# wuqianliang/Diff-Reg

Measured on AMD Instinct MI355X. Metric: scene-pairs/sec @ 20 denoise steps (N=M=256); IR/FMR parity vs ref, higher is better.
Workload: dtype f32; 1 GPU; cfg2: 3DMatch N=M=256, C=432, 20 denoise steps, max_condition_num=200 (warp active), 256 independent B=1 pairs per pass per GPU as 2 concurrent batch(es), one HIP-graph replay each on its own stream; pairs_per_pass_per_gpu=256, streams=2, denoise_steps=20, N=256, M=256, graph=True, parallelism=pairs sharded over 1 GPU(s)

## Files before the change

### diff-reg_amd/csrc/pgemm.hip

```cpp
#include <cstdlib>
#include <string.h>
#include <type_traits>
#include "pgemm.h"

namespace dr {
namespace {

typedef float f32x16 __attribute__((ext_vector_type(16)));
typedef float f32x2 __attribute__((ext_vector_type(2)));
typedef _Float16 f16x8 __attribute__((ext_vector_type(8)));
typedef _Float16 f16x2 __attribute__((ext_vector_type(2)));
typedef unsigned u32x4 __attribute__((ext_vector_type(4)));
typedef __attribute__((address_space(3))) void lds_void;
typedef const __attribute__((address_space(1))) void glb_void;

__device__ __forceinline__ void split2(float x0, float x1, unsigned& hi, unsigned& lo) {
    const f32x2 f = {x0, x1};
    const f16x2 h = __builtin_convertvector(f, f16x2);
    hi = __builtin_bit_cast(unsigned, h);
    const f32x2 hf = __builtin_convertvector(h, f32x2);
    const f32x2 r = {x0 - hf.x, x1 - hf.y};
    lo = __builtin_bit_cast(unsigned, __builtin_convertvector(r, f16x2));
}
__device__ __forceinline__ int scale_exp(float m) {
// ... 133 lines not shown
    const unsigned offBh = A_ST + (wn * BNW + l31) * 64 + ((h ^ sw) << 4), offBl = A_ST + (wn * BNW + l31) * 64 + (((2 + h) ^ sw) << 4);

    f32x16 acc[TNW];
#pragma unroll
    for (int j = 0; j < TNW; ++j)
#pragma unroll
        for (int r = 0; r < 16; ++r) acc[j][r] = 0.f;
    u32x4 fa0[2], fa1[2], fx[TNW / 2][2], fy[TNW - TNW / 2][2];
    f32x4 c16[M16 ? 4 : 1][M16 ? 7 : 1];

    auto run = [&](auto grp_t) __attribute__((always_inline)) {
        constexpr int GRP = decltype(grp_t)::value;
        constexpr bool EARLY = GRP == 0 && NST >= 4;
        constexpr int AHEAD = EARLY ? NST - 2 : NST - 1;
        constexpr bool ALL0 = NST >= 4 && WMN == 4;
        constexpr int AG = ALL0 ? 0 : 1;
        constexpr int WB_CNT = ALL0 ? 0 : (GG::NB + GG::NA) / 2 - GG::NA;
        constexpr int NW0 = GG::NB - WB_CNT;
        constexpr int NAP = GRP == AG ? 2 : 0;
        constexpr int NPIECE = GRP ? NAP + (WB_CNT + WMN - 1) / WMN : NAP + (NW0 + WMN - 1) / WMN;
        constexpr int NFULLP = GRP ? NAP + WB_CNT / WMN : NAP + NW0 / WMN;
        constexpr int PSTEP = (2 * NPIECE <= 3 * (TNW - TNW / 2)) ? 2 : 1;
        static_assert(EARLY || PSTEP * NPIECE <= 3 * (TNW - TNW / 2), "the DMA pieces of a stage must fit the gaps of the second burst");
        static_assert(!EARLY || NPIECE <= 3 * (TNW / 2), "... and those of the early group the gaps of the first");
        constexpr int REMP = GRP ? WB_CNT % WMN : NW0 % WMN;
        const int wl = w % WMN;
        const int st0 = GRP ? wl * (WB_CNT / WMN) + min(wl, WB_CNT % WMN) : WB_CNT + wl * (NW0 / WMN) + min(wl, NW0 % WMN);
        const unsigned voffW = lane * 16 + st0 * 1024, voffA = lane * 16 + 2 * wl * 1024;
        const char* ga = P.A0 + ((size_t)rb128 * P.nc0 + kbeg) * GG::A_IMG + sub * 64;
        const char* gb = P.W.img + ((size_t)nb * (P.nc0 + nc1) + kbeg) * GG::B_ST;
        const char* const ga1 = nc1 > 0 ? P.A1 + (size_t)rb128 * nc1 * GG::A_IMG + sub * 64 : nullptr;
        int ti = 0;
#define PG_DMA(ldsaddr, voff, gbase, imm)                                                                  \
    asm volatile("s_mov_b32 m0, %0\n\ts_nop 0\n\tglobal_load_lds_dwordx4 %1, %2 offset:%3" ::"s"(ldsaddr), "v"(voff), "s"(gbase), "i"(imm) : "memory")
        auto dma_piece = [&](int p, unsigned dstb) __attribute__((always_inline)) {
            const unsigned m0w = dstb + A_ST + st0 * 1024;
            const int pw = p - NAP;
            const unsigned hop = (unsigned)(pw >> 2) * 4096;
            if (p < NAP) PG_DMA(dstb + 2 * wl * 1024, voffA, ga, p * 1024);
            else if (pw < (GRP ? WB_CNT : NW0) / WMN || wl < (GRP ? WB_CNT : NW0) % WMN) PG_DMA(m0w + hop, voffW + hop, gb, (pw & 3) * 1024);
        };
        auto dma_advance = [&]() __attribute__((always_inline)) {
            ++ti;
            gb += GG::B_ST;
            ga = (ti == nc0) ? ga1 : ga + GG::A_IMG;
        };

        auto stage = [&](int s, auto steady_t, u32x4 (&ac)[2], u32x4 (&an)[2]) __attribute__((always_inline)) {
            constexpr bool STEADY = decltype(steady_t)::value;
            constexpr int NT1 = TNW / 2, NT2 = TNW - NT1, M1 = 3 * NT1;
            const unsigned sb = lds_base + (unsigned)(s % NST) * STAGE, sbn = lds_base + (unsigned)((s + 1) % NST) * STAGE;
            const unsigned Bh = sb + offBh, Bl = sb + offBl, Bhn = sbn + offBh, Bln = sbn + offBl;
            const bool has_next = STEADY || s + 1 < nst;
            const bool do_issue = STEADY || ti < nst;
            const unsigned dstb = lds_base + (unsigned)(ti % NST) * STAGE;
            if (s == nc0 && nc1 > 0) {
                const unsigned fb0 = lds_base + GG::WORK + (wm * 32 + 4 * h) * 4;
                u32x4 f[4];
                PG_READ(f[0], fb0, 0); PG_READ(f[1], fb0, 32); PG_READ(f[2], fb0, 64); PG_READ(f[3], fb0, 96);
                asm volatile("s_waitcnt lgkmcnt(0)" ::: "memory");
                __builtin_amdgcn_sched_barrier(0);
#pragma unroll
                for (int j = 0; j < TNW; ++j)
#pragma unroll
                    for (int r = 0; r < 16; ++r) acc[j][r] *= __uint_as_float(f[r >> 2][r & 3]);
                __builtin_amdgcn_sched_barrier(0);
            }
            auto gap = [&](int m) __attribute__((always_inline)) {
                {
                    if (m < NT2) {
                        PG_READ(fy[m][0], Bh, (NT1 + m) * 2048);
                        PG_READ(fy[m][1], Bl, (NT1 + m) * 2048);
                    } else if (m == M1 && has_next) {
                        PG_READ(an[0], sbn + offAh, 0);
                        PG_READ(an[1], sbn + offAl, 0);
                    } else if (m > M1 && m <= M1 + NT1 && has_next) {
                        PG_READ(fx[m - M1 - 1][0], Bhn, (m - M1 - 1) * 2048);
                        PG_READ(fx[m - M1 - 1][1], Bln, (m - M1 - 1) * 2048);
                    }
                }
                constexpr int MF = EARLY ? 0 : (PSTEP == 2 ? M1 + 1 : M1), STEP = EARLY ? 1 : PSTEP;
                if (m >= MF && m < MF + STEP * NPIECE && (m - MF) % STEP == 0) {
                    if (do_issue) dma_piece((m - MF) / STEP, dstb);
                    if ((m - MF) / STEP == NPIECE - 1 && do_issue) dma_advance();
                }
                if (m == M1 - 1) {
                    if (has_next) {
                        if (NST >= 4 && (STEADY || s + 2 < nst)) {
                            if (wl < REMP) PG_VMCNT(NFULLP + 1); else PG_VMCNT(NFULLP);
                        } else {
                            PG_VMCNT(0);
                        }
                    }
                    __builtin_amdgcn_s_barrier();
                    asm volatile("s_waitcnt lgkmcnt(0)" ::: "memory");
                }
            };
            const f16x8 ah = __builtin_bit_cast(f16x8, ac[0]), al = __builtin_bit_cast(f16x8, ac[1]);
#define PG_MFMA(X, Y, g)                                                        \
    acc[j] = __builtin_amdgcn_mfma_f32_32x32x16_f16(X, Y, acc[j], 0, 0, 0);      \
    __builtin_amdgcn_sched_barrier(0);                                          \
    gap(3 * j + g);                                                             \
    __builtin_amdgcn_sched_barrier(0);
            asm volatile("s_waitcnt lgkmcnt(0)" ::: "memory");
            __builtin_amdgcn_sched_barrier(0);
#pragma unroll
            for (int j = 0; j < NT1; ++j) {
                const f16x8 bh = __builtin_bit_cast(f16x8, fx[j][0]), bl = __builtin_bit_cast(f16x8, fx[j][1]);
                PG_MFMA(al, bh, 0)
                PG_MFMA(ah, bl, 1)
                PG_MFMA(ah, bh, 2)
            }
#pragma unroll
            for (int j = NT1; j < TNW; ++j) {
                const f16x8 bh = __builtin_bit_cast(f16x8, fy[j - NT1][0]), bl = __builtin_bit_cast(f16x8, fy[j - NT1][1]);
                PG_MFMA(al, bh, 0)
                PG_MFMA(ah, bl, 1)
                PG_MFMA(ah, bh, 2)
            }
#undef PG_MFMA
        };

#pragma unroll
        for (int q2 = 0; q2 < AHEAD; ++q2) {
            const unsigned dstb = lds_base + (unsigned)q2 * STAGE;
#pragma unroll
            for (int i = 0; i < NPIECE; ++i) dma_piece(i, dstb);
            dma_advance();
            if (q2 == 0) {
                __builtin_amdgcn_sched_barrier(0);
                stage_inputs();
                __builtin_amdgcn_sched_barrier(0);
                PG_VMCNT(0);
            }
        }
        __builtin_amdgcn_s_barrier();
        PG_READ(fa0[0], lds_base + offAh, 0);
        PG_READ(fa0[1], lds_base + offAl, 0);
#pragma unroll
        for (int j = 0; j < TNW / 2; ++j) {
            PG_READ(fx[j][0], lds_base + offBh, j * 2048);
            PG_READ(fx[j][1], lds_base + offBl, j * 2048);
        }
        int s = 0;
        for (; s + 1 < nst - (NST - 1); s += 2) {
            stage(s, std::true_type{}, fa0, fa1);
            stage(s + 1, std::true_type{}, fa1, fa0);
        }
        for (; s < nst; s += 2) {
            stage(s, std::false_type{}, fa0, fa1);
            if (s + 1 < nst) stage(s + 1, std::false_type{}, fa1, fa0);
        }
    };
    auto run16 = [&](auto iss_t) __attribute__((always_inline)) {
        constexpr bool ISS = decltype(iss_t)::value;
        const int l15 = lane & 15, g = lane >> 4, cs = g & 1, uh = g >> 1, sw16 = (l15 >> 2) & 3;
        const int wn4 = w & 3, wm2 = w >> 2;
        const unsigned oAh = cs * STAGE + (wm2 * 64 + l15) * 64 + ((uh ^ sw16) << 4), oAl = cs * STAGE + (wm2 * 64 + l15) * 64 + (((2 + uh) ^ sw16) << 4);
        const unsigned oBh = cs * STAGE + A_ST + (wn4 * 112 + l15) * 64 + ((uh ^ sw16) << 4), oBl = cs * STAGE + A_ST + (wn4 * 112 + l15) * 64 + (((2 + uh) ^ sw16) << 4);
#pragma unroll
        for (int i = 0; i < 4; ++i)
#pragma unroll
            for (int j = 0; j < 7; ++j) c16[i][j] = f32x4{0.f, 0.f, 0.f, 0.f};
        u32x4 fb[7][2], fa[2][2];
        const int nv0 = (nc0 + 1) & ~1, nvt = nv0 + ((nc1 + 1) & ~1), npair = nvt >> 1;
        const int z0 = (nc0 & 1) ? nv0 - 1 : -1, z1 = (nc1 & 1) ? nvt - 1 : -1;
        const int wl = w & 3, st0 = wl * 7;
        const unsigned voffW = lane * 16 + st0 * 1024, voffA = lane * 16 + 2 * wl * 1024;
        const char* ga = P.A0 + (size_t)rb128 * nc0 * GG::A_IMG + sub * 64;
        const char* gb = P.W.img + (size_t)nb * nst * GG::B_ST;
        const char* const ga1 = nc1 > 0 ? P.A1 + (size_t)rb128 * nc1 * GG::A_IMG + sub * 64 : nullptr;
        int ti = 0, tr = 0;
        auto piece = [&](int q) __attribute__((always_inline)) {
            if (ti == z0 || ti == z1) return;
            const unsigned dstb = lds_base + (unsigned)(ti % NST) * STAGE;
            const unsigned m0w = dstb + A_ST + st0 * 1024;
            const int pw = q - 2;
            const unsigned hop = (unsigned)(pw >> 2) * 4096;
            if (q < 2) PG_DMA(dstb + 2 * wl * 1024, voffA, ga, q * 1024);
            else PG_DMA(m0w + hop, voffW + hop, gb, (pw & 3) * 1024);
        };
        auto advance = [&]() __attribute__((always_inline)) {
            if (ti != z0 && ti != z1) {
                ++tr;
                gb += GG::B_ST;
                ga = (tr == nc0) ? ga1 : ga + GG::A_IMG;
            }
            ++ti;
        };
        auto stage = [&](int p, auto steady_t) __attribute__((always_inline)) {
            constexpr bool STEADY = decltype(steady_t)::value;
            const unsigned zm = ((2 * p + 1 == z0 || 2 * p + 1 == z1) && cs) ? 0u : ~0u;
            const unsigned sb = lds_base + (unsigned)(p & 1) * 2 * STAGE, sbn = lds_base + (unsigned)((p + 1) & 1) * 2 * STAGE;
            const bool has_next = STEADY || p + 1 < npair;
            if (2 * p == nv0 && nc1 > 0) {
#pragma unroll
                for (int i = 0; i < 4; ++i) {
                    const float f = s_fac[wm2 * 64 + 16 * i + l15];
#pragma unroll
                    for (int j = 0; j < 7; ++j) c16[i][j] *= f;
                }
                __builtin_amdgcn_sched_barrier(0);
            }
            auto gap = [&](int m) __attribute__((always_inline)) {
                const int pass = m / 21, gi = m % 21;
                if (pass < 3) {
                    if (gi == 0) PG_READ(fa[(pass + 1) & 1][0], sb + oAh, (pass + 1) * 1024);
                    if (gi == 1) PG_READ(fa[(pass + 1) & 1][1], sb + oAl, (pass + 1) * 1024);
                } else if (has_next) {
                    if (gi == 0) PG_READ(fa[0][0], sbn + oAh, 0);
                    if (gi == 1) PG_READ(fa[0][1], sbn + oAl, 0);
                    if (gi >= 1 && gi <= 7) PG_READ(fb[gi - 1][1], sbn + oBl, (gi - 1) * 1024);
                    if (gi >= 15 && gi <= 20) PG_READ(fb[gi - 15][0], sbn + oBh, (gi - 15) * 1024);
                    if (gi == 20) PG_READ(fb[6][0], sbn + oBh, 6 * 1024);
                }
                if (ISS) {
                    if (pass == 3 && gi >= 8 && gi <= 14) {
                        if (STEADY || ti < nvt) piece(gi - 8);
                    }
                    if (pass == 0 && gi % 3 == 2) {
                        const int q = 7 + gi / 3;
                        if (STEADY || ti < nvt) {
                            piece(q < 9 ? q : q - 9);
                            if (q == 8) advance();
                        }
                    }
                    if (pass == 1 && gi % 3 == 2 && gi <= 11) {
                        const int q = 14 + gi / 3;
                        if (STEADY || ti < nvt) {
                            piece(q - 9);
                            if (q == 17) advance();
                        }
                    }
                }
                if (pass == 2 && gi == 17) {
                    if (ISS && has_next) PG_VMCNT(0);
                    __builtin_amdgcn_s_barrier();
                }
            };
#define PG_MFMA16(X, Y, m)                                                              \
    c16[i][j] = __builtin_amdgcn_mfma_f32_16x16x32_f16(Y, X, c16[i][j], 0, 0, 0);       \
    __builtin_amdgcn_sched_barrier(0);                                                  \
    gap(m);                                                                             \
    __builtin_amdgcn_sched_barrier(0);
#pragma unroll
            for (int i = 0; i < 4; ++i) {
                if (i == 0) asm volatile("s_waitcnt lgkmcnt(7)" ::: "memory");
                else asm volatile("s_waitcnt lgkmcnt(0)" ::: "memory");
                __builtin_amdgcn_sched_barrier(0);
                const u32x4 a_h = fa[i & 1][0] & zm, a_l = fa[i & 1][1] & zm;
                const f16x8 ah = __builtin_bit_cast(f16x8, a_h), al = __builtin_bit_cast(f16x8, a_l);
#pragma unroll
                for (int j = 0; j < 7; ++j) { PG_MFMA16(ah, __builtin_bit_cast(f16x8, fb[j][1]), 21 * i + j) }
                if (i == 0) { asm volatile("s_waitcnt lgkmcnt(2)" ::: "memory"); __builtin_amdgcn_sched_barrier(0); }
#pragma unroll
                for (int j = 0; j < 7; ++j) { PG_MFMA16(al, __builtin_bit_cast(f16x8, fb[j][0]), 21 * i + 7 + j) }
#pragma unroll
                for (int j = 0; j < 7; ++j) { PG_MFMA16(ah, __builtin_bit_cast(f16x8, fb[j][0]), 21 * i + 14 + j) }
            }
#undef PG_MFMA16
        };
        if (ISS) {
#pragma unroll
            for (int q = 0; q < 9; ++q) piece(q);
            advance();
#pragma unroll
            for (int q = 0; q < 9; ++q) piece(q);
            advance();
            __builtin_amdgcn_sched_barrier(0);
            stage_inputs();
            __builtin_amdgcn_sched_barrier(0);
            PG_VMCNT(0);
#pragma unroll
            for (int q = 0; q < 7; ++q) piece(q);
        } else {
            stage_inputs();
        }
        __builtin_amdgcn_s_barrier();
        PG_READ(fa[0][0], lds_base + oAh, 0);
        PG_READ(fa[0][1], lds_base + oAl, 0);
#pragma unroll
        for (int j = 0; j < 7; ++j) PG_READ(fb[j][1], lds_base + oBl, j * 1024);
#pragma unroll
        for (int j = 0; j < 7; ++j) PG_READ(fb[j][0], lds_base + oBh, j * 1024);
        int p = 0;
        for (; p < npair - 2; ++p) stage(p, std::true_type{});
        for (; p < npair; ++p) stage(p, std::false_type{});
    };
    if constexpr (M16) {
        if (w < 4) run16(std::true_type{});
        else run16(std::false_type{});
    } else {
        if (wn == 0) run(std::integral_constant<int, 0>{});
        else run(std::integral_constant<int, 1>{});
    }
    if (G.dbg & 1) {
        float keep = 0.f;
        if constexpr (M16) {
#pragma unroll
            for (int i = 0; i < 4; ++i)
#pragma unroll
                for (int j = 0; j < 7; ++j) keep += c16[i][j][0] + c16[i][j][1] + c16[i][j][2] + c16[i][j][3];
        } else {
#pragma unroll
            for (int j = 0; j < TNW; ++j)
#pragma unroll
                for (int r = 0; r < 16; ++r) keep += acc[j][r];
        }
        if (keep == 123.456f && P.out) P.out[0] = keep;
        return;
    }
    __syncthreads();

    int keep = -1;
    if constexpr (KS_OK) {
        if (ksplit) {
            keep = khalf;
            const int give = 1 - khalf;
            int* const s_bad = reinterpret_cast<int*>(s_sum);
            if (t == 0) *s_bad = 0;
            float* const xsend = P.xk_buf + ((((size_t)rb * 2 + give) * 4 + w) * TNW * 2) * 256 + lane * 4;
            const float* const xrecv = P.xk_buf + ((((size_t)rb * 2 + khalf) * 4 + w) * TNW * 2) * 256 + lane * 4;
#pragma unroll
            for (int j = 0; j < TNW; ++j)
#pragma unroll
                for (int q2 = 0; q2 < 2; ++q2) {
                    const f32x4 x = {acc[j][8 * give + 4 * q2], acc[j][8 * give + 4 * q2 + 1], acc[j][8 * give + 4 * q2 + 2], acc[j][8 * give + 4 * q2 + 3]};
                    asm volatile("global_store_dwordx4 %0, %1, off sc0 sc1\n\ts_nop 1" ::"v"(xsend + (j * 2 + q2) * 256), "v"(x) : "memory");
                }
            asm volatile("s_waitcnt vmcnt(0)" ::: "memory");
            __syncthreads();
            unsigned* const fl = P.xk_flags + (size_t)rb * 2;
            if (t == 0) __hip_atomic_store(fl + khalf, P.xk_epoch, __ATOMIC_RELAXED, __HIP_MEMORY_SCOPE_AGENT);
            if (w == 0) {
                unsigned spins = 0;
                while (__hip_atomic_load(fl + give, __ATOMIC_RELAXED, __HIP_MEMORY_SCOPE_AGENT) != P.xk_epoch) {
                    __builtin_amdgcn_s_sleep(1);
                    if (++spins > (1u << 22)) {
                        if (lane == 0) { *s_bad = 1; if (P.xk_status) atomicOr(P.xk_status, 2u); }
                        break;
                    }
                }
            }
            __syncthreads();
            const bool bad = *s_bad != 0;
            f32x4 y[TNW][2];
#pragma unroll
            for (int j = 0; j < TNW; ++j)
#pragma unroll
                for (int q2 = 0; q2 < 2; ++q2)
                    asm volatile("global_load_dwordx4 %0, %1, off sc1" : "=&v"(y[j][q2]) : "v"(xrecv + (j * 2 + q2) * 256) : "memory");
            asm volatile("s_waitcnt vmcnt(0)" ::: "memory");
            __builtin_amdgcn_sched_barrier(0);
            const float poison = bad ? __uint_as_float(0x7fc00000u) : 0.f;
#pragma unroll
            for (int j = 0; j < TNW; ++j)
#pragma unroll
                for (int q2 = 0; q2 < 2; ++q2)
#pragma unroll
                    for (int e = 0; e < 4; ++e) acc[j][8 * khalf + 4 * q2 + e] += y[j][q2][e] + poison;
            __syncthreads();
            if (G.dbg & 64) {
                float kp = 0.f;
#pragma unroll
                for (int j = 0; j < TNW; ++j)
#pragma unroll
                    for (int r = 0; r < 16; ++r) kp += acc[j][r];
                if (kp == 123.456f && P.out) P.out[0] = kp;
                return;
            }
        }
    }
    auto skip = [&](int rr) __attribute__((always_inline)) { return KS_OK && keep >= 0 && rr != keep; };

    const int lr = M16 ? (lane & 15) : (lane >> 2), q = M16 ? (lane >> 4) : (lane & 3);
    constexpr int NR = M16 ? 4 : 2, NIE = M16 ? 7 : NI, EPS = M16 ? 112 : EP_S;
    const int wcol0 = M16 ? (w & 3) * 112 : wn * BNW, wrow0 = M16 ? (w >> 2) * 64 : wm * 32, wcw = M16 ? (w & 3) : wn;
    const int lrow = lr;
    float* const ep = reinterpret_cast<float*>(lds) + w * (16 * EPS);
    float cv[M16 ? 1 : TNW];
    if constexpr (!M16) {
#pragma unroll
        for (int j = 0; j < TNW; ++j) cv[j] = s_cinv[wn * BNW + l31 + 32 * j];
    }
    auto transpose_round = [&](int rr, float4 (&dst)[NIE]) __attribute__((always_inline)) {
        if constexpr (M16) {
            const float rinv = s_rinv[wrow0 + 16 * rr + lrow];
#pragma unroll
            for (int i = 0; i < NIE; ++i) {
                const float4 c4 = *reinterpret_cast<const float4*>(s_cinv + wcol0 + 16 * i + 4 * q);
                const f32x4 a = c16[rr][i];
                dst[i] = make_float4(a[0] * c4.x * rinv, a[1] * c4.y * rinv, a[2] * c4.z * rinv, a[3] * c4.w * rinv);
            }
            return;
        } else {
#pragma unroll
            for (int j = 0; j < TNW; ++j)
#pragma unroll
                for (int r8 = 0; r8 < 8; ++r8) {
                    const int r = 8 * rr + r8;
                    ep[((r & 3) + 8 * ((r >> 2) & 1) + 4 * h) * EPS + 32 * j + l31] = acc[j][r] * cv[j];
                }
        }
        wave_fence();
        const float rinv = s_rinv[wrow0 + 16 * rr + lrow];
#pragma unroll
        for (int i = 0; i < NIE; ++i) {
            float4 x = *reinterpret_cast<const float4*>(ep + lr * EPS + 16 * i + 4 * q);
            x.x *= rinv; x.y *= rinv; x.z *= rinv; x.w *= rinv;
            dst[i] = x;
        }
        wave_fence();
    };
    const int colw = wcol0 + 4 * q;
    auto add_bias = [&](float4 (&dst)[NIE]) __attribute__((always_inline)) {
        if (has_bias) {
#pragma unroll
            for (int i = 0; i < NIE; ++i) {
                const float4 b4 = *reinterpret_cast<const float4*>(s_bias + colw + 16 * i);
                dst[i].x += b4.x; dst[i].y += b4.y; dst[i].z += b4.z; dst[i].w += b4.w;
            }
        }
    };
    int grow[NR];
#pragma unroll
    for (int rr = 0; rr < NR; ++rr) grow[rr] = rb * BM + wrow0 + 16 * rr + lrow;
    constexpr int mode = MODE;

    float4 v[NR][NIE];
    auto row_sum4 = [&](float s) __attribute__((always_inline)) {
        if constexpr (M16) {
            typedef unsigned u32x2 __attribute__((ext_vector_type(2)));
            const unsigned u = __float_as_uint(s);
            const u32x2 a = __builtin_amdgcn_permlane16_swap(u, u, false, false);
            const float t2 = __uint_as_float(a.x) + __uint_as_float(a.y);
            const unsigned w2 = __float_as_uint(t2);
            const u32x2 b = __builtin_amdgcn_permlane32_swap(w2, w2, false, false);
            return __uint_as_float(b.x) + __uint_as_float(b.y);
        } else {
            s += dpp_xor1f(s);
            s += dpp_xor2f(s);
            return s;
        }
    };
    if (mode != PG_LN) {
        const int halfC = P.rot_C >> 1, rpad = P.rot_piece_pad, rlen = P.rot_piece_len;
        const unsigned rmagic = rpad > 0 ? ((1u << 20) + rpad - 1) / rpad : 0u;
        const float scale = P.scale;
#define PG_TABLE_INDEX(i)                                                                                                   \
    int col = min(colw + 16 * (i), C - 4);                                                                                  \
    if (rpad > 0) { const int hq = (int)(((unsigned)col * rmagic) >> 20); col = hq * rlen + min(col - hq * rpad, rlen - 4); } \
    if (col >= P.rot_C) col %= P.rot_C;                     \
    const int ridx = col >> 1;
#define PG_LOAD_TABLES(rr, tb)                                                                                              \
    {                                                                                                                       \
    if (P.csT) {                                          \
        const float* pp = P.csT + (size_t)min(grow[rr], rows - 1) * halfC * 2;                                              \
        _Pragma("unroll") for (int i = 0; i < NIE; ++i) {                                                                   \
            PG_TABLE_INDEX(i)                                                                                               \
            const float4 cs = *reinterpret_cast<const float4*>(pp + 2 * ridx);                                              \
            tb[i] = make_float4(cs.x, cs.z, cs.y, cs.w);                                                                    \
        }                                                                                                                   \
    } else {                                                                                                                \
        const float* cp = P.cosT + (size_t)min(grow[rr], rows - 1) * halfC;                                                 \
        const float* sp = P.sinT + (size_t)min(grow[rr], rows - 1) * halfC;                                                 \
        _Pragma("unroll") for (int i = 0; i < NIE; ++i) {                                                                   \
            PG_TABLE_INDEX(i)                                                                                               \
            const float2 c = *reinterpret_cast<const float2*>(cp + ridx), sn = *reinterpret_cast<const float2*>(sp + ridx); \
            tb[i] = make_float4(c.x, c.y, sn.x, sn.y);                                                                      \
        }                                                                                                                   \
    }                                                                                                                       \
    }
        auto finish_round = [&](int rr, const float4 (&tb)[NIE]) __attribute__((always_inline)) {
            add_bias(v[rr]);
#pragma unroll
            for (int i = 0; i < NIE; ++i) {
                float4 x = v[rr][i];
                if (rot) {
                    const float x0 = x.x, x1 = x.y, x2 = x.z, x3 = x.w;
                    x.x = __fadd_rn(__fmul_rn(x0, tb[i].x), __fmul_rn(-x1, tb[i].z));
                    x.y = __fadd_rn(__fmul_rn(x1, tb[i].x), __fmul_rn(x0, tb[i].z));
                    x.z = __fadd_rn(__fmul_rn(x2, tb[i].y), __fmul_rn(-x3, tb[i].w));
                    x.w = __fadd_rn(__fmul_rn(x3, tb[i].y), __fmul_rn(x2, tb[i].w));
                }
                x.x *= scale; x.y *= scale; x.z *= scale; x.w *= scale;
                if (mode == PG_PLANES && P.relu) { x.x = fmaxf(x.x, 0.f); x.y = fmaxf(x.y, 0.f); x.z = fmaxf(x.z, 0.f); x.w = fmaxf(x.w, 0.f); }
                v[rr][i] = x;
            }
        };
        if constexpr (!M16) {
#pragma unroll
            for (int rr = 0; rr < NR; ++rr) {
                float4 tb[NIE];
                if (rot && !(G.dbg & 32)) PG_LOAD_TABLES(rr, tb)
                transpose_round(rr, v[rr]);
                finish_round(rr, tb);
                __builtin_amdgcn_sched_barrier(0);
            }
        } else {
            float4 tb0[NIE], tb1[NIE];
            if (rot && !(G.dbg & 32)) { PG_LOAD_TABLES(0, tb0) PG_LOAD_TABLES(1, tb1) }
            transpose_round(0, v[0]);
            transpose_round(1, v[1]);
            finish_round(0, tb0);
            __builtin_amdgcn_sched_barrier(0);
            if (rot && !(G.dbg & 32)) PG_LOAD_TABLES(2, tb0)
            finish_round(1, tb1);
            __builtin_amdgcn_sched_barrier(0);
            if (rot && !(G.dbg & 32)) PG_LOAD_TABLES(3, tb1)
            transpose_round(2, v[2]);
            transpose_round(3, v[3]);
            finish_round(2, tb0);
            finish_round(3, tb1);
            __builtin_amdgcn_sched_barrier(0);
        }
#undef PG_LOAD_TABLES
#undef PG_TABLE_INDEX
        if (mode == PG_F32) {
            float* __restrict__ outp = P.out + (size_t)nb * P.blk_stride;
#pragma unroll
            for (int rr = 0; rr < NR; ++rr) {
                if (grow[rr] >= rows) continue;
#pragma unroll
                for (int i = 0; i < NIE; ++i) {
                    const int col = colw + 16 * i;
                    if (wcol0 + 16 * i < C && !(G.dbg & 4)) *reinterpret_cast<float4*>(outp + (size_t)grow[rr] * P.ldo + col) = v[rr][i];
                }
            }
            return;
        }
        if (mode == PG_PLANES && P.out) {
            float* __restrict__ outp = P.out + (size_t)nb * P.blk_stride;
#pragma unroll
            for (int rr = 0; rr < NR; ++rr) {
                if (grow[rr] >= rows) continue;
#pragma unroll
                for (int i = 0; i < NIE; ++i) {
                    const int col = colw + 16 * i;
                    if (wcol0 + 16 * i < C && !(G.dbg & 4)) *reinterpret_cast<float4*>(outp + (size_t)grow[rr] * P.ldo + col) = v[rr][i];
                }
            }
        }
    } else {
#pragma unroll
        for (int rr = 0; rr < NR; ++rr) if (!skip(rr)) transpose_round(rr, v[rr]);
#pragma unroll
        for (int rr = 0; rr < NR; ++rr) if (!skip(rr)) add_bias(v[rr]);
    }

    if (mode == PG_LN) {
        const float* __restrict__ res = P.resid;
        constexpr int NRR = NR / 2;
        float4 r0[NRR][NIE];
        auto park = [&](int rr) __attribute__((always_inline)) { return ep + (rr - NRR) * (8 * 16 * EPS) + lr * EPS + 4 * q; };
        if (res && !(G.dbg & 16)) {
#pragma unroll
            for (int rr = NRR; rr < NR; ++rr) {
                if (skip(rr)) continue;
                const float* rp = res + (size_t)min(grow[rr], rows - 1) * P.ldr;
#pragma unroll
                for (int i = 0; i < NIE; ++i) {
                    const int col = colw + 16 * i;
                    const float4 x = wcol0 + 16 * i < C ? *reinterpret_cast<const float4*>(rp + col) : make_float4(0.f, 0.f, 0.f, 0.f);
                    *reinterpret_cast<float4*>(park(rr) + 16 * i) = x;
                }
            }
#pragma unroll
            for (int rr = 0; rr < NRR; ++rr) {
                if (skip(rr)) continue;
                const float* rp = res + (size_t)min(grow[rr], rows - 1) * P.ldr;
#pragma unroll
                for (int i = 0; i < NIE; ++i) {
                    const int col = colw + 16 * i;
                    r0[rr][i] = wcol0 + 16 * i < C ? *reinterpret_cast<const float4*>(rp + col) : make_float4(0.f, 0.f, 0.f, 0.f);
                }
            }
        }
        const bool postadd = res && P.ln_postadd;
        if (postadd) {
#pragma unroll
            for (int rr = 0; rr < NR; ++rr)
#pragma unroll
                for (int i = 0; i < NIE; ++i) {
                    if (skip(rr)) continue;
                    const float4 r4 = rr < NRR ? r0[rr < NRR ? rr : 0][i] : *reinterpret_cast<const float4*>(park(rr) + 16 * i);
                    v[rr][i].x += r4.x; v[rr][i].y += r4.y; v[rr][i].z += r4.z; v[rr][i].w += r4.w;
                }
        }
        float mean[NR], rstd[NR];
#pragma unroll
        for (int rr = 0; rr < NR; ++rr) {
            if (skip(rr)) continue;
            float s = 0.f;
#pragma unroll
            for (int i = 0; i < NIE; ++i)
                if (wcol0 + 16 * i < C) s += (v[rr][i].x + v[rr][i].y) + (v[rr][i].z + v[rr][i].w);
            s = row_sum4(s);
            if (q == 0) s_sum[wcw * 128 + wrow0 + 16 * rr + lrow] = s;
        }
        __syncthreads();
#pragma unroll
        for (int rr = 0; rr < NR; ++rr) {
            if (skip(rr)) continue;
            const int rl = wrow0 + 16 * rr + lrow;
            float tot = s_sum[rl];
#pragma unroll
            for (int c = 1; c < NCW; ++c) tot += s_sum[c * 128 + rl];
            mean[rr] = tot / (float)C;
            float s = 0.f;
#pragma unroll
            for (int i = 0; i < NIE; ++i)
                if (wcol0 + 16 * i < C) {
                    const float d0 = v[rr][i].x - mean[rr], d1 = v[rr][i].y - mean[rr], d2 = v[rr][i].z - mean[rr], d3 = v[rr][i].w - mean[rr];
                    s = fmaf(d0, d0, s); s = fmaf(d1, d1, s); s = fmaf(d2, d2, s); s = fmaf(d3, d3, s);
                }
            s = row_sum4(s);
            if (q == 0) s_sq[wcw * 128 + rl] = s;
        }
        __syncthreads();
#pragma unroll
        for (int rr = 0; rr < NR; ++rr) {
            if (skip(rr)) continue;
            const int rl = wrow0 + 16 * rr + lrow;
            float tot = s_sq[rl];
#pragma unroll
            for (int c = 1; c < NCW; ++c) tot += s_sq[c * 128 + rl];
            rstd[rr] = 1.0f / sqrtf(tot / (float)C + 1e-5f);
            const bool rok = grow[rr] < rows;
#pragma unroll
            for (int i = 0; i < NIE; ++i) {
                const int col = colw + 16 * i;
                if (wcol0 + 16 * i < C) {
                    const float4 g4 = *reinterpret_cast<const float4*>(s_gam + col), b4 = *reinterpret_cast<const float4*>(s_bet + col);
                    float4 y;
                    y.x = (v[rr][i].x - mean[rr]) * rstd[rr] * g4.x + b4.x; y.y = (v[rr][i].y - mean[rr]) * rstd[rr] * g4.y + b4.y;
                    y.z = (v[rr][i].z - mean[rr]) * rstd[rr] * g4.z + b4.z; y.w = (v[rr][i].w - mean[rr]) * rstd[rr] * g4.w + b4.w;
                    if (res && !postadd) {
                        const float4 r4 = rr < NRR ? r0[rr < NRR ? rr : 0][i] : *reinterpret_cast<const float4*>(park(rr) + 16 * i);
                        y.x += r4.x; y.y += r4.y; y.z += r4.z; y.w += r4.w;
                    }
                    v[rr][i] = y;
                    if (P.out && rok && !(G.dbg & 4)) *reinterpret_cast<float4*>(P.out + (size_t)grow[rr] * P.ldo + col) = y;
                }
            }
        }
    }
    if (!P.pimg) return;

#pragma unroll
    for (int rr = 0; rr < NR; ++rr) {
        if (skip(rr)) continue;
        const bool rok = grow[rr] < rows;
        const float bound = s_bound[wrow0 + 16 * rr + lrow];
        if (P.pbnd && rok && (nb == 0 || per_blk) && wcw == 0 && q == 0) P.pbnd[(size_t)nb * P.pbnd_blk_stride + grow[rr]] = bound;
        const float sc = pow2i(scale_exp(bound));
        const int rl = sub + wrow0 + 16 * rr + lrow, swz = (rl >> 2) & 3;
        char* const rowp = P.pimg + (size_t)nb * P.pimg_blk_stride +
                           (((size_t)rb128 * P.p_nct + P.p_kc0 + (per_blk ? 0 : nb * (C >> 4)) + (wcol0 >> 4)) * 128 + rl) * 64;
        const unsigned uh = (unsigned)(((q >> 1) ^ swz) << 4), ul = (unsigned)(((2 + (q >> 1)) ^ swz) << 4);
#pragma unroll
        for (int i = 0; i < NIE; ++i) {
            if (wcol0 + 16 * i >= C) continue;
// ... 535 lines not shown
            split2(v[g][0].x * sc, v[g][0].y * sc, hi.x, lo.x); split2(v[g][0].z * sc, v[g][0].w * sc, hi.y, lo.y);
            split2(v[g][1].x * sc, v[g][1].y * sc, hi.z, lo.z); split2(v[g][1].z * sc, v[g][1].w * sc, hi.w, lo.w);
            char* d = img + (((size_t)rb * nct + (gi >> 1)) * 128 + r) * 64;
            *reinterpret_cast<uint4*>(d + (((gi & 1) ^ swz) << 4)) = hi;
            *reinterpret_cast<uint4*>(d + (((2 + (gi & 1)) ^ swz) << 4)) = lo;
        }
    }
}
__global__ __launch_bounds__(256) void planes_to_f32_kernel(const char* __restrict__ img, const float* __restrict__ bnd, int rows, int K,
                                                            float* __restrict__ out, int ldo) {
    const int row = blockIdx.x * 4 + (threadIdx.x >> 6), lane = threadIdx.x & 63;
    if (row >= rows) return;
    const int ng = K >> 3, nct = K >> 4, rb = row >> 7, r = row & 127, swz = (r >> 2) & 3;
    const float inv = pow2i(-scale_exp(bnd[row]));
    for (int gi = lane; gi < ng; gi += 64) {
        const char* d = img + (((size_t)rb * nct + (gi >> 1)) * 128 + r) * 64;
        const f16x8 hi = *reinterpret_cast<const f16x8*>(d + (((gi & 1) ^ swz) << 4));
        const f16x8 lo = *reinterpret_cast<const f16x8*>(d + (((2 + (gi & 1)) ^ swz) << 4));
#pragma unroll
        for (int e = 0; e < 8; ++e) out[(size_t)row * ldo + 8 * gi + e] = ((float)hi[e] + (float)lo[e]) * inv;
    }
}
__global__ __launch_bounds__(256) void ln_bound_kernel(const float* __restrict__ g, const float* __restrict__ b, int C, float* __restrict__ out) {
    __shared__ float sg[4], sb[4];
    float mg = 0.f, mb = 0.f;
    for (int c = threadIdx.x; c < C; c += 256) { mg = fmaxf(mg, fabsf(g[c])); mb = fmaxf(mb, fabsf(b[c])); }
    mg = wave_max(mg); mb = wave_max(mb);
    if ((threadIdx.x & 63) == 0) { sg[threadIdx.x >> 6] = mg; sb[threadIdx.x >> 6] = mb; }
    __syncthreads();
    if (threadIdx.x == 0) {
        mg = fmaxf(fmaxf(sg[0], sg[1]), fmaxf(sg[2], sg[3]));
        mb = fmaxf(fmaxf(sb[0], sb[1]), fmaxf(sb[2], sb[3]));
        out[0] = (sqrtf((float)C) * mg + mb) * 1.0001f;
    }
}

using G4 = PgGeom<4, 4>;
using G4H = PgGeom<4, 4, 2>;
using G7 = PgGeom<7, 4>;
using G9 = PgGeom<9, 3>;
using G7H = PgGeom<7, 4, 2>;
using G9H = PgGeom<9, 3, 2>;

}

bool pgemm_shape_ok(int C) { return C > 0 && C % 16 == 0 && C <= G9::BN; }
int pgemm_bn(int C) { return C <= G4::BN ? G4::BN : (C <= G7::BN ? G7::BN : G9::BN); }
static size_t pg_bst(int C) { return (size_t)pgemm_bn(C) * 64; }

template <int TNW, int NST, int MODE>
static int configure_mode() {
    if constexpr (TNW <= 7)
        DR_HIP_CHECK(hipFuncSetAttribute((const void*)pgemm_kernel<TNW, NST, MODE, 4>, hipFuncAttributeMaxDynamicSharedMemorySize, (int)PgGeom<TNW, NST, 4>::SMEM));
    if constexpr (TNW == 7) {
        DR_HIP_CHECK(hipFuncSetAttribute((const void*)pgemm_kernel<TNW, NST, MODE, 4, true>, hipFuncAttributeMaxDynamicSharedMemorySize, (int)PgGeom<TNW, NST, 4>::SMEM16));
    }
    DR_HIP_CHECK(hipFuncSetAttribute((const void*)pgemm_kernel<TNW, NST, MODE, 2>, hipFuncAttributeMaxDynamicSharedMemorySize, (int)PgGeom<TNW, NST, 2>::SMEM));
    return DR_OK;
}
int pgemm_configure() {
    int rc = configure_mode<4, 4, PG_F32>();
    if (rc == DR_OK) rc = configure_mode<4, 4, PG_PLANES>();
    if (rc == DR_OK) rc = configure_mode<4, 4, PG_LN>();
    if (rc == DR_OK) rc = configure_mode<7, 4, PG_F32>();
    if (rc == DR_OK) rc = configure_mode<7, 4, PG_PLANES>();
    if (rc == DR_OK) rc = configure_mode<7, 4, PG_LN>();
    if (rc == DR_OK) rc = configure_mode<9, 3, PG_F32>();
    if (rc == DR_OK) rc = configure_mode<9, 3, PG_PLANES>();
    if (rc == DR_OK) rc = configure_mode<9, 3, PG_LN>();
    if (rc == DR_OK) {
        DR_HIP_CHECK(hipFuncSetAttribute((const void*)pgemm16w_kernel<PG_F32>, hipFuncAttributeMaxDynamicSharedMemorySize, (int)PgGeomW::SMEM));
        DR_HIP_CHECK(hipFuncSetAttribute((const void*)pgemm16w_kernel<PG_PLANES>, hipFuncAttributeMaxDynamicSharedMemorySize, (int)PgGeomW::SMEM));
    }
    return rc;
}

template <int TNW, int NST, int WMN>
static void pg_launch(int mode, dim3 grid, hipStream_t st, const PgBatch& g) {
    using GG = PgGeom<TNW, NST, WMN>;
    if (mode == PG_F32) hipLaunchKernelGGL((pgemm_kernel<TNW, NST, PG_F32, WMN>), grid, dim3(GG::NTHR), GG::SMEM, st, g);
    else if (mode == PG_PLANES) hipLaunchKernelGGL((pgemm_kernel<TNW, NST, PG_PLANES, WMN>), grid, dim3(GG::NTHR), GG::SMEM, st, g);
    else hipLaunchKernelGGL((pgemm_kernel<TNW, NST, PG_LN, WMN>), grid, dim3(GG::NTHR), GG::SMEM, st, g);
}

static int launch_pgemm16w(const PgBatch& g, hipStream_t st) {
    int maxt = 0;
    double flops = 0;
    const int mode = g.p[0].mode;
    if (mode != PG_F32 && mode != PG_PLANES) return DR_ENOSUP;
    bool ksplit = env_knob("DR_PG_KSPLIT", 1) != 0 && env_knob("DR_PG_KSPLITW", 1) != 0;
    long tiles = 0;
    for (int i = 0; i < g.n; ++i) {
        const PgProblem& p = g.p[i];
        const long tl_ = (long)((p.rows + 127) / 128) * p.nblk * 2;
        ksplit = ksplit && p.xk_buf && p.xk_flags && tl_ <= p.xk_cap && (p.A1 ? (p.nc0 >= 5 && p.nc1 >= 5) : p.nc0 >= 12);
        tiles += tl_;
    }
    ksplit = ksplit && 2 * tiles <= (long)device_cu_count();
    for (int i = 0; i < g.n; ++i) {
        const PgProblem& p = g.p[i];
        const int nst = p.nc0 + (p.A1 ? p.nc1 : 0);
        if (p.W.sub != 2 || !pgemm16w_shape_ok(p.C) || p.rows < 1 || p.nblk < 1 || p.nc0 < 5 || (p.A1 && p.nc1 < 5) || p.mode != mode) return DR_ENOSUP;
        if (p.W.nct != nst) return DR_EINVAL;
        const int tl = ((p.rows + 127) / 128 + 7) / 8 * 8 * p.nblk * 2 * (ksplit ? 2 : 1);
        maxt = tl > maxt ? tl : maxt;
        flops += 2.0 * p.rows * p.C * p.nblk * (p.k_alg > 0 ? (double)p.k_alg : 16.0 * p.W.nct);
    }
    ProfScope ps(PK_GEMM_SPLIT, flops, st);
    PgBatch gd = g;
    gd.dbg = env_knob("DR_PG_NOEPI", 0);
    for (int i = 0; i < g.n; ++i) gd.p[i].ksplit = ksplit ? 1 : 0;
    const dim3 grid(maxt, g.n);
    if (mode == PG_F32) hipLaunchKernelGGL((pgemm16w_kernel<PG_F32>), grid, dim3(PgGeomW::NTHR), PgGeomW::SMEM, st, gd);
    else hipLaunchKernelGGL((pgemm16w_kernel<PG_PLANES>), grid, dim3(PgGeomW::NTHR), PgGeomW::SMEM, st, gd);
    DR_LAUNCH_CHECK();
    return DR_OK;
}

int launch_pgemm(const PgBatch& g, hipStream_t st) {
    if (g.n < 1 || g.n > 3) return DR_EINVAL;
    if (g.p[0].W.sub == 2) return launch_pgemm16w(g, st);
    int maxt = 0;
    double flops = 0;
    const int bn = pgemm_bn(g.p[0].C), nst_min = bn == G9::BN ? G9::NST : G7::NST;
    const int half_env = env_knob("DR_PG_HALF", 1);
    const int n_cu = device_cu_count();
    long wg128 = 0;
    for (int i = 0; i < g.n; ++i) wg128 += (long)((g.p[i].rows + 127) / 128) * g.p[i].nblk;
    const bool half = bn == G9::BN || half_env == 2 || (half_env == 1 && wg128 * 100 < (long)n_cu * env_knob("DR_PG_HALF_PCT", 51));
    const int bm = half ? 64 : 128;
    bool ksplit = half && g.p[0].mode == PG_LN && env_knob("DR_PG_KSPLIT", 1) != 0;
    long wg64 = 0;
    for (int i = 0; i < g.n; ++i) {
        const PgProblem& p = g.p[i];
        const long rb64 = (p.rows + 63) / 64;
        ksplit = ksplit && p.xk_buf && p.xk_flags && p.nblk == 1 && !p.A1 && p.nc0 / 2 >= nst_min && rb64 <= p.xk_cap;
        wg64 += rb64;
    }
    ksplit = ksplit && 2 * wg64 <= (long)n_cu;
    for (int i = 0; i < g.n; ++i) {
        const PgProblem& p = g.p[i];
        if (!pgemm_shape_ok(p.C) || pgemm_bn(p.C) != bn || p.rows < 1 || p.nblk < 1 || p.nc0 < 1 || p.nc0 + (p.A1 ? p.nc1 : 0) < nst_min) return DR_ENOSUP;
        if (p.W.nct != p.nc0 + (p.A1 ? p.nc1 : 0)) return DR_EINVAL;
        const int tl = ((p.rows + bm - 1) / bm + 7) / 8 * 8 * (ksplit ? 2 : p.nblk);
        maxt = tl > maxt ? tl : maxt;
        flops += 2.0 * p.rows * p.C * p.nblk * (p.k_alg > 0 ? (double)p.k_alg : 16.0 * p.W.nct);
    }
    ProfScope ps(PK_GEMM_SPLIT, flops, st);
    const int mode = g.p[0].mode;
    for (int i = 1; i < g.n; ++i)
        if (g.p[i].mode != mode) return DR_EINVAL;
    const dim3 grid(maxt, g.n);
    PgBatch gd = g;
    gd.dbg = env_knob("DR_PG_NOEPI", 0);
    for (int i = 0; i < g.n; ++i) gd.p[i].ksplit = ksplit ? 1 : 0;
    if (bn == G9::BN) pg_launch<9, 3, 2>(mode, grid, st, gd);
    else if (bn == G4::BN) { if (half) pg_launch<4, 4, 2>(mode, grid, st, gd); else pg_launch<4, 4, 4>(mode, grid, st, gd); }
    else {
        bool m16 = env_knob("DR_PG_M16", 1) != 0;
        for (int i = 0; i < g.n; ++i) m16 = m16 && g.p[i].nc0 >= 5 && (!g.p[i].A1 || g.p[i].nc1 >= 5);
        if (half) pg_launch<7, 4, 2>(mode, grid, st, gd);
        else if (m16) {
            using GG = PgGeom<7, 4, 4>;
            if (mode == PG_F32) hipLaunchKernelGGL((pgemm_kernel<7, 4, PG_F32, 4, true>), grid, dim3(GG::NTHR), GG::SMEM16, st, gd);
            else if (mode == PG_PLANES) hipLaunchKernelGGL((pgemm_kernel<7, 4, PG_PLANES, 4, true>), grid, dim3(GG::NTHR), GG::SMEM16, st, gd);
            else hipLaunchKernelGGL((pgemm_kernel<7, 4, PG_LN, 4, true>), grid, dim3(GG::NTHR), GG::SMEM16, st, gd);
        } else pg_launch<7, 4, 4>(mode, grid, st, gd);
    }
    DR_LAUNCH_CHECK();
    return DR_OK;
}

size_t pgemm_weight_bytes(int C, int nblk, int nct) {
    size_t b = (size_t)nblk * nct * pg_bst(C);
    b += (size_t)nblk * pgemm_bn(C) * 4;
    b += (size_t)nblk * 4;
    return (b + 255) & ~(size_t)255;
}
void pgemm_weight_view(void* buf, int C, int nblk, int nct, PgW* v) {
    char* p = (char*)buf;
    v->img = p;
    v->cinv = reinterpret_cast<const float*>(p + (size_t)nblk * nct * pg_bst(C));
    v->wnorm = v->cinv + (size_t)nblk * pgemm_bn(C);
    v->nct = nct;
    v->sub = 0;
}

bool pgemm16w_shape_ok(int C) { return C > 0 && C % 16 == 0 && C <= PgGeomW::LBN; }
size_t pgemm16w_weight_bytes(int nblk, int nct) {
    size_t b = (size_t)nblk * 2 * nct * PgGeomW::B_ST + (size_t)nblk * PgGeomW::LBN * 4 + (size_t)nblk * 4;
    return (b + 255) & ~(size_t)255;
}
void pgemm16w_weight_view(void* buf, int nblk, int nct, PgW* v) {
    char* p = (char*)buf;
    v->img = p;
    v->cinv = reinterpret_cast<const float*>(p + (size_t)nblk * 2 * nct * PgGeomW::B_ST);
    v->wnorm = v->cinv + (size_t)nblk * PgGeomW::LBN;
    v->nct = nct;
    v->sub = 2;
}
int pgemm16w_pack_weights_block(const float* W, int C, int K, int piece_len, int piece_pad, const PgW& v, int nb, hipStream_t st, int out_len,
                                int out_pad) {
    const int olen = out_len > 0 ? out_len : C, opad = out_pad > 0 ? out_pad : C, rows_src = out_len > 0 ? C / opad * olen : C;
    if (!pgemm16w_shape_ok(C) || v.sub != 2 || piece_pad % 16 || piece_len > piece_pad || piece_len < 1) return DR_EINVAL;
    const int nct = (K + piece_len - 1) / piece_len * piece_pad / 16;
    if (nct != v.nct) return DR_EINVAL;
    constexpr int LBN = PgGeomW::LBN;
    float* cinv = (float*)v.cinv + (size_t)nb * LBN;
    float* wnorm = (float*)v.wnorm + nb;
    char* img = (char*)v.img + (size_t)nb * 2 * nct * PgGeomW::B_ST;
    DR_HIP_CHECK(hipMemsetAsync(wnorm, 0, 4, st));
    hipLaunchKernelGGL(pg_wscale_kernel, dim3((LBN + 3) / 4), dim3(256), 0, st, W, 1, C, K, LBN, cinv, wnorm, olen, opad, rows_src);
    DR_LAUNCH_CHECK();
    const size_t n = (size_t)2 * nct * PgGeomW::BN * 2;
    hipLaunchKernelGGL(pg_pack16w_kernel, dim3((unsigned)((n + 255) / 256)), dim3(256), 0, st, W, 1, C, K, nct, piece_len, piece_pad,
                       (const float*)cinv, img, olen, opad, rows_src);
    DR_LAUNCH_CHECK();
    return DR_OK;
}
int pgemm_pack_weights(const float* W, int nblk, int C, int K, int piece_len, int piece_pad, void* buf, hipStream_t st) {
    if (!pgemm_shape_ok(C) || piece_pad % 16 || piece_len > piece_pad || piece_len < 1) return DR_EINVAL;
    const int nct = (K + piece_len - 1) / piece_len * piece_pad / 16, BN = pgemm_bn(C);
    PgW v;
    pgemm_weight_view(buf, C, nblk, nct, &v);
    DR_HIP_CHECK(hipMemsetAsync((void*)v.wnorm, 0, (size_t)nblk * 4, st));
    hipLaunchKernelGGL(pg_wscale_kernel, dim3((nblk * BN + 3) / 4), dim3(256), 0, st, W, nblk, C, K, BN, (float*)v.cinv, (float*)v.wnorm, C, C, C);
    DR_LAUNCH_CHECK();
    const size_t n = (size_t)nblk * nct * BN * 2;
    hipLaunchKernelGGL(pg_pack_kernel, dim3((unsigned)((n + 255) / 256)), dim3(256), 0, st, W, nblk, C, K, BN, nct, piece_len, piece_pad,
                       v.cinv, (char*)v.img, C, C, C);
    DR_LAUNCH_CHECK();
    return DR_OK;
}

int pgemm_pack_weights_block(const float* W, int C, int K, int piece_len, int piece_pad, const PgW& v, int nb, hipStream_t st, int out_len,
                             int out_pad) {
    const int olen = out_len > 0 ? out_len : C, opad = out_pad > 0 ? out_pad : C, rows_src = out_len > 0 ? C / opad * olen : C;
    if (!pgemm_shape_ok(C) || piece_pad % 16 || piece_len > piece_pad || piece_len < 1) return DR_EINVAL;
    const int nct = (K + piece_len - 1) / piece_len * piece_pad / 16;
    if (nct != v.nct) return DR_EINVAL;
    const int BN = pgemm_bn(C);
    float* cinv = (float*)v.cinv + (size_t)nb * BN;
    float* wnorm = (float*)v.wnorm + nb;
    char* img = (char*)v.img + (size_t)nb * nct * pg_bst(C);
    DR_HIP_CHECK(hipMemsetAsync(wnorm, 0, 4, st));
    hipLaunchKernelGGL(pg_wscale_kernel, dim3((BN + 3) / 4), dim3(256), 0, st, W, 1, C, K, BN, cinv, wnorm, olen, opad, rows_src);
    DR_LAUNCH_CHECK();
    const size_t n = (size_t)nct * BN * 2;
    hipLaunchKernelGGL(pg_pack_kernel, dim3((unsigned)((n + 255) / 256)), dim3(256), 0, st, W, 1, C, K, BN, nct, piece_len, piece_pad,
                       (const float*)cinv, img, olen, opad, rows_src);
    DR_LAUNCH_CHECK();
    return DR_OK;
}

__global__ __launch_bounds__(256) void group_max_kernel(const float* __restrict__ bnd, int ngroups, int grp_rows, float* __restrict__ out) {
    const int g = blockIdx.x * 4 + (threadIdx.x >> 6), lane = threadIdx.x & 63;
    if (g >= ngroups) return;
    float m = 0.f;
    for (int r = lane; r < grp_rows; r += 64) m = fmaxf(m, bnd[(size_t)g * grp_rows + r]);
    m = wave_max(m);
    if (lane == 0) out[g] = m;
}
int launch_group_max(const float* bnd, int ngroups, int grp_rows, float* out, hipStream_t st) {
    if (ngroups < 1) return DR_OK;
    hipLaunchKernelGGL(group_max_kernel, dim3((ngroups + 3) / 4), dim3(256), 0, st, bnd, ngroups, grp_rows, out);
    DR_LAUNCH_CHECK();
    return DR_OK;
}

int launch_planes_from_f32(const float* x, int ldx, int rows, int K, char* img, float* bnd, hipStream_t st, const float* bnd_in) {
    if (K % 16 || K > 1024 || ldx % 4 || ((uintptr_t)x & 15)) return DR_ENOSUP;
    if (rows < 1) return DR_OK;
    hipLaunchKernelGGL(planes_from_f32_kernel, dim3((rows + 3) / 4), dim3(256), 0, st, x, ldx, rows, K, img, bnd, bnd_in);
    DR_LAUNCH_CHECK();
    return DR_OK;
}
int launch_planes_to_f32(const char* img, const float* bnd, int rows, int K, float* out, int ldo, hipStream_t st) {
    if (K % 16) return DR_ENOSUP;
    if (rows < 1) return DR_OK;
    hipLaunchKernelGGL(planes_to_f32_kernel, dim3((rows + 3) / 4), dim3(256), 0, st, img, bnd, rows, K, out, ldo);
    DR_LAUNCH_CHECK();
    return DR_OK;
}
__global__ __launch_bounds__(256) void absmax_blocks_kernel(const float* __restrict__ x, int n, float* __restrict__ out) {
    __shared__ float sm[4];
    const float* xb = x + (size_t)blockIdx.x * n;
    float m = 0.f;
    for (int c = threadIdx.x; c < n; c += 256) m = fmaxf(m, fabsf(xb[c]));
    m = wave_max(m);
    if ((threadIdx.x & 63) == 0) sm[threadIdx.x >> 6] = m;
    __syncthreads();
    if (threadIdx.x == 0) out[blockIdx.x] = fmaxf(fmaxf(sm[0], sm[1]), fmaxf(sm[2], sm[3])) * 1.0001f;
}
int launch_absmax_blocks(const float* x, int nblk, int n, float* out, hipStream_t st) {
    if (nblk < 1) return DR_OK;
    hipLaunchKernelGGL(absmax_blocks_kernel, dim3(nblk), dim3(256), 0, st, x, n, out);
    DR_LAUNCH_CHECK();
    return DR_OK;
}
int launch_ln_bound(const float* gamma, const float* beta, int C, float* out, hipStream_t st) {
    hipLaunchKernelGGL(ln_bound_kernel, dim3(1), dim3(256), 0, st, gamma, beta, C, out);
    DR_LAUNCH_CHECK();
    return DR_OK;
}

}

// ... 145 lines not shown
```

Before: 1190 pairs/s.

## Prefetch epilogue rotation tables into LDS during final GEMM stage

In the M16 GEMM kernel, the rotation cos/sin tables needed by the epilogue are now DMA'd into LDS during the last K-pipeline stage, interleaved into MFMA gaps. The remaining pieces are issued after the first two rounds are consumed. This hides the global-load latency of the table fetch behind compute instead of stalling the epilogue. It adds vmcnt accounting and LDS slot reuse that must stay consistent with the stage buffers, and it can be disabled with an env knob.

```diff
diff --git a/diff-reg_amd/csrc/pgemm.hip b/diff-reg_amd/csrc/pgemm.hip
--- a/diff-reg_amd/csrc/pgemm.hip
+++ b/diff-reg_amd/csrc/pgemm.hip
@@ -309,6 +309,34 @@
             if (s + 1 < nst) stage(s + 1, std::false_type{}, fa1, fa0);
         }
     };
+    constexpr bool PF_OK = M16 && WMN == 4;
+    const bool pf_rot = PF_OK && MODE != PG_LN && rot && P.csT != nullptr && !(G.dbg & (32 | 128));
+    const bool pf = pf_rot;
+    const int pf_npair = (((nc0 + 1) & ~1) + ((nc1 + 1) & ~1)) >> 1;
+    const unsigned pf_off[2] = {(unsigned)(pf_npair & 1) * 2 * STAGE + w * 9216, (unsigned)((pf_npair - 1) & 1) * 2 * STAGE + w * 9216};
+    auto pf_slot = [&](int k) __attribute__((always_inline)) {
+        const int s = k % 18;
+        return pf_off[s / 9] + (unsigned)(s % 9) * 1024;
+    };
+    auto pf_issue = [&](int k) __attribute__((always_inline)) {
+        const int rr = k / 7, i = k % 7;
+        const int rloc = min((w >> 2) * 64 + 16 * rr + (lane & 15), rows - 1 - rb * BM);
+        int col = min((w & 3) * 112 + 4 * (lane >> 4) + 16 * i, C - 4);
+        const int halfC = P.rot_C >> 1, rpad = P.rot_piece_pad, rlen = P.rot_piece_len;
+        if (rpad > 0) {
+            const unsigned rmagic = ((1u << 20) + rpad - 1) / rpad;
+            const int hq = (int)(((unsigned)col * rmagic) >> 20);
+            col = hq * rlen + min(col - hq * rpad, rlen - 4);
+        }
+        if (col >= P.rot_C) col %= P.rot_C;
+        const unsigned voff = (unsigned)(rloc * halfC * 2 + (col >> 1) * 2) * 4;
+        const char* const base = reinterpret_cast<const char*>(P.csT + (size_t)rb * BM * halfC * 2);
+        PG_DMA(lds_base + pf_slot(k), voff, base, 0);
+    };
+    auto pf_piece = [&](int k) __attribute__((always_inline)) {
+        return *reinterpret_cast<const float4*>(lds + pf_slot(k) + lane * 16);
+    };
+
     auto run16 = [&](auto iss_t) __attribute__((always_inline)) {
         constexpr bool ISS = decltype(iss_t)::value;
         const int l15 = lane & 15, g = lane >> 4, cs = g & 1, uh = g >> 1, sw16 = (l15 >> 2) & 3;
@@ -350,6 +378,7 @@
             const unsigned zm = ((2 * p + 1 == z0 || 2 * p + 1 == z1) && cs) ? 0u : ~0u;
             const unsigned sb = lds_base + (unsigned)(p & 1) * 2 * STAGE, sbn = lds_base + (unsigned)((p + 1) & 1) * 2 * STAGE;
             const bool has_next = STEADY || p + 1 < npair;
+            const bool pf_now = !STEADY && pf && p + 1 == npair;
             if (2 * p == nv0 && nc1 > 0) {
 #pragma unroll
                 for (int i = 0; i < 4; ++i) {
@@ -390,6 +419,9 @@
                         }
                     }
                 }
+                if (!STEADY && (pass == 0 || pass == 3) && gi >= 2 && gi <= 18 && gi % 2 == 0) {
+                    if (pf_now) pf_issue((pass == 0 ? 0 : 9) + gi / 2 - 1);
+                }
                 if (pass == 2 && gi == 17) {
                     if (ISS && has_next) PG_VMCNT(0);
                     __builtin_amdgcn_s_barrier();
@@ -465,6 +497,7 @@
                 for (int r = 0; r < 16; ++r) keep += acc[j][r];
         }
         if (keep == 123.456f && P.out) P.out[0] = keep;
+        if (pf) PG_VMCNT(0);
         return;
     }
     __syncthreads();
@@ -656,15 +689,35 @@
             }
         } else {
             float4 tb0[NIE], tb1[NIE];
-            if (rot && !(G.dbg & 32)) { PG_LOAD_TABLES(0, tb0) PG_LOAD_TABLES(1, tb1) }
+            auto pf_tables = [&](int rr, float4 (&tb)[NIE]) __attribute__((always_inline)) {
+#pragma unroll
+                for (int i = 0; i < NIE; ++i) {
+                    const float4 cs = pf_piece(7 * rr + i);
+                    tb[i] = make_float4(cs.x, cs.z, cs.y, cs.w);
+                }
+            };
+            if constexpr (PF_OK) {
+                if (pf_rot) {
+                    PG_VMCNT(4);
+                    pf_tables(0, tb0);
+                    pf_tables(1, tb1);
+                    asm volatile("s_waitcnt lgkmcnt(0)" ::: "memory");
+                    __builtin_amdgcn_sched_barrier(0);
+#pragma unroll
+                    for (int k = 18; k < 28; ++k) pf_issue(k);
+                }
+            }
+            if (rot && !(G.dbg & 32) && !pf_rot) { PG_LOAD_TABLES(0, tb0) PG_LOAD_TABLES(1, tb1) }
             transpose_round(0, v[0]);
             transpose_round(1, v[1]);
             finish_round(0, tb0);
             __builtin_amdgcn_sched_barrier(0);
-            if (rot && !(G.dbg & 32)) PG_LOAD_TABLES(2, tb0)
+            if (pf_rot) { PG_VMCNT(7); pf_tables(2, tb0); }
+            else if (rot && !(G.dbg & 32)) PG_LOAD_TABLES(2, tb0)
             finish_round(1, tb1);
             __builtin_amdgcn_sched_barrier(0);
-            if (rot && !(G.dbg & 32)) PG_LOAD_TABLES(3, tb1)
+            if (pf_rot) { PG_VMCNT(0); pf_tables(3, tb1); }
+            else if (rot && !(G.dbg & 32)) PG_LOAD_TABLES(3, tb1)
             transpose_round(2, v[2]);
             transpose_round(3, v[3]);
             finish_round(2, tb0);
@@ -1506,7 +1559,7 @@
         if (g.p[i].mode != mode) return DR_EINVAL;
     const dim3 grid(maxt, g.n);
     PgBatch gd = g;
-    gd.dbg = env_knob("DR_PG_NOEPI", 0);
+    gd.dbg = env_knob("DR_PG_NOEPI", 0) | (env_knob("DR_PG_EPI_PREFETCH", 1) != 0 ? 0 : 128);
     for (int i = 0; i < g.n; ++i) gd.p[i].ksplit = ksplit ? 1 : 0;
     if (bn == G9::BN) pg_launch<9, 3, 2>(mode, grid, st, gd);
     else if (bn == G4::BN) { if (half) pg_launch<4, 4, 2>(mode, grid, st, gd); else pg_launch<4, 4, 4>(mode, grid, st, gd); }
```

After: 1174 pairs/s. -1.3%, worse.
